# arkworks-rs/algebra

Hardware: AMD Instinct MI355X
Metric: G1 scalar-muls/sec (MSM, 2^24) (higher is better)
Workload: dtype u32

## Files before the change

algebra_amd/_lib.py:

```python
import ctypes as C
import os

_HERE = os.path.dirname(os.path.abspath(__file__))
LIB_PATH = os.environ.get("ARK_HIP_LIB") or os.path.join(_HERE, "libark_hip.so")

u64p = C.POINTER(C.c_uint64)


class ArkHipError(RuntimeError):
    def __init__(self, code, what):
        super().__init__("%s failed with code %d" % (what, code))
        self.code = code


class Radix2DomainStruct(C.Structure):
    _fields_ = [
        ("size", C.c_uint64),
        ("log_size_of_group", C.c_uint32),
        ("_pad", C.c_uint32),
        ("size_as_field_element", C.c_uint64 * 4),
        ("size_inv", C.c_uint64 * 4),
        ("group_gen", C.c_uint64 * 4),
        ("group_gen_inv", C.c_uint64 * 4),
        ("offset", C.c_uint64 * 4),
# ... 131 lines not shown
    "ark_hip_test_host_sw_check": (C.c_int, [C.c_int, C.c_void_p, C.c_size_t, C.c_int, C.c_int, C.c_void_p]),
    "ark_hip_test_host_sw_decompress": (C.c_int, [C.c_int, C.c_void_p, C.c_size_t, C.c_int, C.c_int, C.c_void_p, C.c_void_p]),
    "ark_hip_test_host_sw_compress": (C.c_int, [C.c_int, C.c_void_p, C.c_size_t, C.c_void_p]),
    "ark_hip_test_host_sw_mul": (C.c_int, [C.c_int, C.c_void_p, C.c_int, C.c_void_p, C.c_size_t, C.c_int, C.c_int, C.c_size_t, C.c_void_p]),
    "ark_hip_test_host_sw_add": (C.c_int, [C.c_int, C.c_void_p, C.c_void_p, C.c_int, C.c_size_t, C.c_void_p]),
    "ark_hip_test_host_sw_fold": (C.c_int, [C.c_int, C.c_void_p, C.c_void_p, C.c_int, C.c_void_p, C.c_void_p, C.c_int, C.c_int, C.c_size_t,
                                            C.c_void_p]),
    "ark_hip_test_coord_sqrt": (C.c_int, [C.c_int, C.c_void_p, C.c_void_p, C.c_void_p, C.c_size_t]),
    "ark_hip_test_host_coord_sqrt": (C.c_int, [C.c_int, C.c_void_p, C.c_void_p, C.c_void_p, C.c_size_t]),
    "ark_hip_test_point_op": (C.c_int, [C.c_int, C.c_int, C.c_void_p, C.c_void_p, C.c_void_p, C.c_size_t]),
    "ark_hip_test_msm_sharded_emulated": (C.c_int, [C.c_int, C.c_int, C.POINTER(C.c_void_p), C.POINTER(C.c_void_p),
                                                    C.POINTER(C.c_size_t), C.c_int, C.c_void_p, C.POINTER(C.c_int)]),
    "ark_hip_test_base_hash": (C.c_int, [C.c_void_p, C.c_size_t, C.POINTER(C.c_uint64)]),
    "ark_hip_test_lazy_raw_op": (C.c_int, [C.c_int, C.c_int, C.c_int, C.c_int, C.c_void_p, C.c_void_p, C.c_size_t]),
    "ark_hip_test_lazy_acc_op": (C.c_int, [C.c_int, C.c_int, C.c_void_p, C.c_void_p, C.c_void_p, C.c_size_t]),
    "ark_hip_test_relaxed_raw_op": (C.c_int, [C.c_int, C.c_int, C.c_void_p, C.c_void_p, C.c_size_t]),
    "ark_hip_test_relaxed_acc_op": (C.c_int, [C.c_int, C.c_int, C.c_void_p, C.c_void_p, C.c_void_p, C.c_size_t]),
    "ark_hip_test_msm_host_fold": (C.c_int, [C.c_int, C.c_void_p, C.c_int, C.c_int, C.c_int, C.c_void_p, C.c_void_p]),
    "ark_hip_test_msm_reduce_geometry": (C.c_int, [C.c_int, C.c_int, C.c_int, C.c_int, C.c_int, C.c_size_t, C.POINTER(C.c_uint32)]),
    "ark_hip_test_msm_sort_geometry": (C.c_int, [C.c_int, C.c_size_t, C.c_int, C.c_int, C.c_int, C.c_int, C.POINTER(C.c_int32),
                                                 C.POINTER(C.c_uint64)]),
    "ark_hip_test_msm_sort_stages": (C.c_int, [C.c_int, C.c_void_p, C.c_int, C.c_size_t, C.c_int, C.c_int, C.c_int,
                                               C.POINTER(C.c_int32), C.POINTER(C.c_uint64), C.POINTER(C.c_void_p),
                                               C.POINTER(C.c_size_t)]),
    "ark_hip_test_msm_pieces": (C.c_int, [C.c_int, C.c_void_p, C.c_void_p, C.c_int, C.c_size_t, C.c_int, C.POINTER(C.c_size_t), C.c_int,
                                          C.POINTER(C.c_int32), C.POINTER(C.c_uint64), C.c_void_p, C.c_size_t, C.c_void_p, C.c_size_t,
                                          C.c_void_p]),
    "ark_hip_test_msm_host_fold_l0": (C.c_int, [C.c_int, C.c_void_p, C.c_int, C.c_int, C.c_int, C.c_void_p, C.c_void_p]),
}

# ... 66 lines not shown
```

algebra_amd/csrc/curve_consts.hpp:

```cpp
#pragma once
#include <stdint.h>
namespace arkhip {
static const uint64_t GEN_BN254_G1[8] = {0xd35d438dc58f0d9dULL, 0x0a78eb28f5c70b3dULL, 0x666ea36f7879462cULL, 0x0e0a77c19a07df2fULL, 0xa6ba871b8b1e1b3aULL, 0x14f1d651eb8e167bULL, 0xccdd46def0f28c58ULL, 0x1c14ef83340fbe5eULL};
static const uint64_t GEN_BLS12_381_G1[12] = {0x5cb38790fd530c16ULL, 0x7817fc679976fff5ULL, 0x154f95c7143ba1c1ULL, 0xf0ae6acdf3d0e747ULL, 0xedce6ecc21dbf440ULL, 0x120177419e0bfb75ULL, 0xbaac93d50ce72271ULL, 0x8c22631a7918fd8eULL, 0xdd595f13570725ceULL, 0x51ac582950405194ULL, 0x0e1c8c3fad0059c0ULL, 0x0bbc3efc5008a26aULL};
static const uint64_t GEN_BLS12_377_G1[12] = {0x260f33b9772451f4ULL, 0xc54dd773169d5658ULL, 0x5c1551c469a510ddULL, 0x761662e4425e1698ULL, 0xc97d78cc6f065272ULL, 0x00a41206b361fd4dULL, 0x8193961fb8cb81f3ULL, 0x00638d4c5f44adb8ULL, 0xfafaf3dad4daf54aULL, 0xc27849e2d655cd18ULL, 0x2ec3ddb401d52814ULL, 0x007da93326303c71ULL};
static const uint64_t GEN_BLS12_377_G2[24] = {0x68904082f268725bULL, 0x668f2ea74f45328bULL, 0xebca7a65802be84fULL, 0x1e1850f4c1ada3e6ULL, 0x830dc22d588ef1e9ULL, 0x01862a81767c0982ULL, 0x5f02a915c91c7f39ULL, 0xf8c553ba388da2a7ULL, 0xd51a416dbd198850ULL, 0xe943c6f38ae3073aULL, 0xffe24aa8259a4981ULL, 0x011853391e73dfddULL, 0xd5b19b897881430fULL, 0x05be9118a5b371edULL, 0x6063f91f86c131eeULL, 0x3244a61be8f4ec19ULL, 0xa02e425b9f9a3a12ULL, 0x018af8c04f3360d2ULL, 0x57601ac71a5b96f5ULL, 0xe99acc1714f2440eULL, 0x2339612f10118ea9ULL, 0x8321e68a3b1cd722ULL, 0x2b543b050cc74917ULL, 0x00590182b396c112ULL};
static const uint64_t GEN_BLS12_381_G2[24] = {0xf5f28fa202940a10ULL, 0xb3f5fb2687b4961aULL, 0xa1a893b53e2ae580ULL, 0x9894999d1a3caee9ULL, 0x6f67b7631863366bULL, 0x058191924350bcd7ULL, 0xa5a9c0759e23f606ULL, 0xaaa0c59dbccd60c3ULL, 0x3bb17e18e2867806ULL, 0x1b1ab6cc8541b367ULL, 0xc2b6ed0ef2158547ULL, 0x11922a097360edf3ULL, 0x4c730af860494c4aULL, 0x597cfa1f5e369c5aULL, 0xe7e6856caa0a635aULL, 0xbbefb5e96e0d495fULL, 0x07d3a975f0ef25a2ULL, 0x0083fd8e7e80dae5ULL, 0xadc0fc92df64b05dULL, 0x18aa270a2b1461dcULL, 0x86adac6a3be4eba0ULL, 0x79495c4ec93da33aULL, 0xe7175850a43ccaedULL, 0x0b2bc2a163de1bf2ULL};
}
```

algebra_amd/csrc/lazyk.cuh:

```cuda
#pragma once
#include "curves.cuh"
#include "ec28.cuh"
#include "ec28x2.cuh"

namespace arkhip {

template <class C, int LANES_ = C::FA::LANES>
struct LazyK;

template <class C>
struct LazyK<C, 1> {
  typedef typename C::F FM;
  typedef typename FM::P P;
  typedef FpL<P> FL;
  typedef XYZZL<P> Acc;
  static constexpr u32 LANES = 1;
  static constexpr int WORDS = 4 * FL::L + 1;
  ARK_HD static Acc inf() {
    Acc a;
    a.inf = true;
    a.x = a.y = a.zz = a.zzz = FL::zero();
    return a;
  }
  ARK_HD static Acc from_bucket(const XYZZ<FM>& b) { return lazy_from_bucket<P>(b); }
// ... 24 lines not shown
    const u32* w = (const u32*)slot;
    Acc a;
#pragma unroll
    for (int i = 0; i < FL::L; i++) {
      a.x.l[i] = w[i];
      a.y.l[i] = w[FL::L + i];
      a.zz.l[i] = w[2 * FL::L + i];
      a.zzz.l[i] = w[3 * FL::L + i];
    }
    a.inf = w[4 * FL::L] != 0u;
    return a;
  }
};

template <class C>
struct LazyK<C, 2> {
  typedef typename C::FA FM;
  typedef typename FM::P P;
  typedef Fp2L<P, FM::NEG_BETA_> FL;
  typedef XYZZL2<FL> Acc;
  static constexpr u32 LANES = 2;
  static constexpr int L = FL::L;
  static constexpr int WORDS = 8 * L + 1;
  ARK_DEV static Acc inf() { return lazy2_inf<FL>(); }
  ARK_DEV static Acc from_bucket(const XYZZ<FM>& b) { return lazy2_from_bucket<FL>(b); }
  ARK_DEV static XYZZ<FM> to_bucket(const Acc& a) { return lazy2_to_bucket<FL>(a); }
  ARK_DEV static bool madd(Acc& acc, const Affine<FM>& p, bool neg) {
    return xyzz_madd_lazy2<FL>(acc, FL::from_canonical(p.x), FL::from_canonical(FM::cond_neg(p.y, neg)));
  }
  ARK_DEV static void mdbl(Acc& out, const char* src, bool neg) { lazy2_mdbl<FL>(out, src, neg); }
// ... 33 lines not shown
```

algebra_amd/csrc/msm.cuh:

```cuda
#pragma once
#include <hip/hip_runtime.h>
#include <stdio.h>
#include <stdlib.h>
#include <vector>
#include <mutex>
#include <atomic>
#include "hostpool.hpp"
#include <math.h>
#include "curves.cuh"
#include "ec28.cuh"
#include "lazyk.cuh"
#include "msm_sort.cuh"
#include "msm_plan.hpp"

namespace arkhip {

#define ARK_HIP_TRY(expr)                                                                          \
  do {                                                                                             \
    hipError_t _e = (expr);                                                                        \
    if (_e != hipSuccess) {                                                                        \
      fprintf(stderr, "ark_hip: %s failed: %s (%s:%d)\n", #expr, hipGetErrorString(_e), __FILE__, __LINE__); \
      return -(int)_e - 1000;                                                                      \
    }                                                                                              \
  } while (0)
// ... 441 lines not shown
  }
  if constexpr (C::RELAXED_A) acc = xyzz_canonical<F>(acc);
  acc.store(cell);
}

#ifndef ARK_LAZY_MIN_WAVES
#define ARK_LAZY_MIN_WAVES 2
#endif
template <class C>
__global__ void __launch_bounds__(256, ARK_LAZY_MIN_WAVES) msm_accumulate_lazy_kernel(const char* __restrict__ bases,
                                                                  const u32* __restrict__ sorted,
                                                                  const u32* __restrict__ offsets,
                                                                  const u32* __restrict__ order, u32 nbuckets,
                                                                  const u32* __restrict__ d_thresh, int HB, int LB,
                                                                  int accum, char* __restrict__ buckets) {
  typedef LazyK<C> K;
  typedef typename K::FM F;
  u32 t = (blockIdx.x * blockDim.x + threadIdx.x) / K::LANES;
  if (t >= nbuckets) return;
  u32 g = order ? order[t] : t;
  u32 j = offsets[g], end = offsets[g + 1];
  if (end - j > *d_thresh) return;
  if (accum && j == end) return;
  char* cell = buckets + (size_t)msm_slot_to_bucket(g, HB, LB) * XYZZ<F>::BYTES;
  typename K::Acc acc = K::inf();
  if (accum) acc = K::from_bucket(XYZZ<F>::load(cell));
  if (j < end) {
    u32 e = sorted[j];
    u32 e1 = j + 1 < end ? sorted[j + 1] : 0;
    Affine<F> p = Affine<F>::load(bases + (size_t)(e & 0x7fffffffu) * Affine<F>::BYTES);
    for (;;) {
// ... 1494 lines not shown
```

algebra_amd/csrc/testops_curve.hip:

```cpp
#include "devops.cuh"
#include "testops.cuh"
#include "lazytest.cuh"
#include "relaxtest.cuh"
#include "pointcodec.cuh"
#include "internal.hpp"
#ifndef ARK_TEST_CURVE
#error "compile with -DARK_TEST_CURVE=BLS12_381_G1 (or another curve of curves.cuh)"
#endif
#define ARK_CAT2(a, b) a##b
#define ARK_CAT(a, b) ARK_CAT2(a, b)
namespace arkhip {
int ARK_CAT(test_basefield_op_, ARK_TEST_CURVE)(int op, const void* a, const void* b, void* r, size_t n, hipStream_t s) {
  return field_op_launch<ARK_TEST_CURVE::F, false>(op, a, b, r, n, s);
}
int ARK_CAT(test_point_op_, ARK_TEST_CURVE)(int kind, const void* acc, const void* other, void* out, size_t n, hipStream_t s) {
  return test_point_op_launch<ARK_TEST_CURVE>(kind, acc, other, out, n, s);
}
int ARK_CAT(test_coord_sqrt_, ARK_TEST_CURVE)(const void* in, void* out, void* ok, size_t n, hipStream_t s) {
  return coord_sqrt_launch<ARK_TEST_CURVE>(in, out, ok, n, s);
}
int ARK_CAT(test_lazy_raw_op_, ARK_TEST_CURVE)(int op, int k, int h, const void* in, void* out, size_t n, hipStream_t s) {
  typedef LazyK<ARK_TEST_CURVE> K;
  if constexpr (K::LANES == 1) return lazytest::lazy_raw_op_launch<typename K::P, false, void>(op, k, h, in, out, n, s);
  else return lazytest::lazy_raw_op_launch<typename K::P, false, typename K::FL>(op, k, h, in, out, n, s);
}
int ARK_CAT(test_lazy_acc_op_, ARK_TEST_CURVE)(int kind, const void* acc, const void* other, void* out, size_t n, hipStream_t s) {
  return lazytest::lazy_acc_op_launch<ARK_TEST_CURVE>(kind, acc, other, out, n, s);
}
int ARK_CAT(test_relaxed_raw_op_, ARK_TEST_CURVE)(int op, const void* in, void* out, size_t n, hipStream_t s) {
  typedef ARK_TEST_CURVE::FA FA;
  return relaxtest::relaxed_raw_op_launch<FA::P, relaxtest::NegBetaOf<FA>::v>(op, in, out, n, s);
}
int ARK_CAT(test_relaxed_acc_op_, ARK_TEST_CURVE)(int kind, const void* acc, const void* other, void* out, size_t n, hipStream_t s) {
  return relaxtest::relaxed_acc_op_launch<ARK_TEST_CURVE>(kind, acc, other, out, n, s);
}
}
```

algebra_amd/csrc/ubench/issuebench.hip:

```cpp
#include <hip/hip_runtime.h>
#include <stdint.h>
#include <stdio.h>
typedef uint32_t u32;
typedef uint64_t u64;

#define R8(X) X X X X X X X X
#define KERNEL32(NAME, I0, I1, I2, I3)                                                                        \
  __global__ void __launch_bounds__(256) NAME(u64* out, int iters) {                                         \
    u32 tid = blockIdx.x * blockDim.x + threadIdx.x;                                                          \
    u32 a0 = tid, a1 = tid + 1, a2 = tid + 2, a3 = tid + 3;                                                   \
    const u32 x = tid * 2654435761u | 0x80000001u, y = (tid * 40503u + 7u) | 0x80000000u;                     \
    for (int k = 0; k < iters; k++)                                                                           \
      asm volatile(R8(I0 "\n\t" I1 "\n\t" I2 "\n\t" I3 "\n\t") : "+v"(a0), "+v"(a1), "+v"(a2), "+v"(a3) : "v"(x), "v"(y) : "vcc"); \
    out[tid] = a0 ^ a1 ^ a2 ^ a3;                                                                             \
  }
#define KERNEL64(NAME, T, TX, I0, I1, I2, I3)                                                                     \
  __global__ void __launch_bounds__(256) NAME(u64* out, int iters) {                                         \
    u32 tid = blockIdx.x * blockDim.x + threadIdx.x;                                                          \
    T a0 = (T)tid, a1 = (T)(tid + 1), a2 = (T)(tid + 2), a3 = (T)(tid + 3);                                   \
    const TX x = (TX)(tid | 1u), y = (TX)((tid * 40503u + 7u) | 0x80000000u);                                    \
    for (int k = 0; k < iters; k++)                                                                           \
      asm volatile(R8(I0 "\n\t" I1 "\n\t" I2 "\n\t" I3 "\n\t") : "+v"(a0), "+v"(a1), "+v"(a2), "+v"(a3) : "v"(x), "v"(y) : "vcc"); \
    T s = a0 + a1 + a2 + a3;                                                                                  \
    out[tid] = *(u64*)&s;                                                                                     \
  }
KERNEL32(k_add32, "v_add_u32 %0, %4, %0", "v_add_u32 %1, %4, %1", "v_add_u32 %2, %4, %2", "v_add_u32 %3, %4, %3")
KERNEL32(k_mad24, "v_mad_u32_u24 %0, %4, %5, %0", "v_mad_u32_u24 %1, %4, %5, %1", "v_mad_u32_u24 %2, %4, %5, %2", "v_mad_u32_u24 %3, %4, %5, %3")
KERNEL32(k_mulhi24, "v_mul_hi_u32_u24 %0, %4, %0", "v_mul_hi_u32_u24 %1, %4, %1", "v_mul_hi_u32_u24 %2, %4, %2", "v_mul_hi_u32_u24 %3, %4, %3")
KERNEL32(k_mullo32, "v_mul_lo_u32 %0, %4, %0", "v_mul_lo_u32 %1, %4, %1", "v_mul_lo_u32 %2, %4, %2", "v_mul_lo_u32 %3, %4, %3")
KERNEL32(k_mulhi32, "v_mul_hi_u32 %0, %4, %0", "v_mul_hi_u32 %1, %4, %1", "v_mul_hi_u32 %2, %4, %2", "v_mul_hi_u32 %3, %4, %3")
KERNEL32(k_addc, "v_add_co_u32 %0, vcc, %4, %0", "v_addc_co_u32 %1, vcc, %5, %1, vcc", "v_add_co_u32 %2, vcc, %4, %2", "v_addc_co_u32 %3, vcc, %5, %3, vcc")
KERNEL64(k_mad64, u64, u32, "v_mad_u64_u32 %0, vcc, %4, %5, %0", "v_mad_u64_u32 %1, vcc, %4, %5, %1", "v_mad_u64_u32 %2, vcc, %4, %5, %2", "v_mad_u64_u32 %3, vcc, %4, %5, %3")
KERNEL64(k_add64, u64, u64, "v_lshl_add_u64 %0, %4, 0, %0", "v_lshl_add_u64 %1, %4, 0, %1", "v_lshl_add_u64 %2, %4, 0, %2", "v_lshl_add_u64 %3, %4, 0, %3")
KERNEL64(k_fma64, double, double, "v_fma_f64 %0, %4, %5, %0", "v_fma_f64 %1, %4, %5, %1", "v_fma_f64 %2, %4, %5, %2", "v_fma_f64 %3, %4, %5, %3")
KERNEL64(k_mul64f, double, double, "v_mul_f64 %0, %4, %0", "v_mul_f64 %1, %4, %1", "v_mul_f64 %2, %4, %2", "v_mul_f64 %3, %4, %3")

typedef void (*kern_t)(u64*, int);
int main() {
  u64* out;
  if (hipMalloc(&out, 256 * 8 * 256 * 8) != hipSuccess) return 1;
  hipEvent_t e0, e1;
  hipEventCreate(&e0);
  hipEventCreate(&e1);
  struct { const char* name; kern_t k; } ks[] = {
      {"v_add_u32            ", k_add32},  {"v_mad_u32_u24        ", k_mad24},   {"v_mul_hi_u32_u24     ", k_mulhi24},
      {"v_mul_lo_u32         ", k_mullo32}, {"v_mul_hi_u32         ", k_mulhi32}, {"v_add_co + v_addc_co ", k_addc},
      {"v_mad_u64_u32        ", k_mad64},  {"v_lshl_add_u64       ", k_add64},   {"v_fma_f64            ", k_fma64},
      {"v_mul_f64            ", k_mul64f}};
  for (auto& e : ks) {
    for (int w : {2, 8}) {
      const int b = 256 * w, it = 4000;
      hipLaunchKernelGGL(e.k, dim3(b), dim3(256), 0, 0, out, 10);
      hipDeviceSynchronize();
      hipEventRecord(e0);
      hipLaunchKernelGGL(e.k, dim3(b), dim3(256), 0, 0, out, it);
      hipEventRecord(e1);
      hipEventSynchronize(e1);
      float ms;
      hipEventElapsedTime(&ms, e0, e1);
      const double rate = (double)b * 256 * it * 32 / (ms * 1e-3);
      printf("%s waves/SIMD=%d  %8.3f ms  %7.2f T lane-ops/s  = %5.2f cycles per wave instruction at 2.4 GHz\n", e.name, w, ms,
             rate * 1e-12, 256.0 * 4 * 64 * 2.4e9 / rate);
// ... 5 lines not shown
```

algebra_amd/csrc/ubench/mulbench.hip:

```cpp
#include "../fp28.cuh"
#include <stdio.h>
using namespace arkhip;
#ifndef MULBENCH_FIELD
#define MULBENCH_FIELD BLS12_381_FQ
#endif
typedef MULBENCH_FIELD P;
template <int V> __global__ void __launch_bounds__(256) k_lazy(u32* out, int iters) {
  typedef FpL<P> L;
  L a, b;
  u32 tid = blockIdx.x * blockDim.x + threadIdx.x;
  for (int i = 0; i < L::L; i++) { a.l[i] = (tid * 2654435761u * (i + 1)) & L::MASK; b.l[i] = ((tid ^ 77) * 40503u * (i + 3)) & L::MASK; }
  a.l[L::L - 1] &= 0xfff; b.l[L::L - 1] &= 0xfff;
  for (int k = 0; k < iters; k++) {
    if constexpr (V == 0) a = L::mul_c(a, b);
    else if constexpr (V == 1) a = L::mul(a, b);
    else if constexpr (V == 2) a = L::sqr(a);
    else if constexpr (V == 3) a = L::sop2(a, b, b, a);
    else a = L::sqr_c(a);
  }
  u32 r = 0;
  for (int i = 0; i < L::L; i++) r ^= a.l[i];
  out[tid] = r;
}
__global__ void __launch_bounds__(256) k_sat(u32* out, int iters) {
  typedef Fp<P> F;
  F a, b;
  u32 tid = blockIdx.x * blockDim.x + threadIdx.x;
  for (int i = 0; i < F::N; i++) { a.l[i] = (tid * 2654435761u * (i + 1)); b.l[i] = ((tid ^ 77) * 40503u * (i + 3)); }
  a.l[F::N - 1] &= 0x7ffffff; b.l[F::N - 1] &= 0x7ffffff;
  for (int k = 0; k < iters; k++) a = F::mul(a, b);
  u32 r = 0;
  for (int i = 0; i < F::N; i++) r ^= a.l[i];
  out[tid] = r;
}
__global__ void __launch_bounds__(256) k_mad_peak(u64* out, int iters, u32 mask) {
  u32 tid = blockIdx.x * blockDim.x + threadIdx.x;
  u64 a0 = tid, a1 = tid + 1, a2 = tid + 2, a3 = tid + 3;
  const u32 x = (tid * 2654435761u | 0x80000001u) & mask, y = ((tid * 40503u + 7u) | 0x80000000u) & mask;
// ... 38 lines not shown
          case 4: hipLaunchKernelGGL((k_lazy<4>), dim3(b), dim3(256), 0, 0, out, it); break;
          default: hipLaunchKernelGGL(k_sat, dim3(b), dim3(256), 0, 0, out, it);
        }
      };
      launch(10);
      hipDeviceSynchronize();
      hipEventRecord(e0);
      launch(iters);
      hipEventRecord(e1);
      hipEventSynchronize(e1);
      float ms;
      hipEventElapsedTime(&ms, e0, e1);
      printf("%s waves/SIMD=%d  %8.3f ms  %8.2f G/s\n", names[v], w, ms, (double)b * 256 * iters / (ms * 1e-3) * 1e-9);
    }
  }
  return 0;
}
```

include/ark_hip.h:

```cpp
#ifndef ARK_HIP_H
#define ARK_HIP_H
#include <stddef.h>
#include <stdint.h>
#ifdef __cplusplus
extern "C" {
#endif
#if defined(__GNUC__) || defined(__clang__)
#pragma GCC visibility push(default)
#endif

enum { ARK_HIP_BN254_FQ = 0, ARK_HIP_BN254_FR = 1, ARK_HIP_BLS12_381_FQ = 2, ARK_HIP_BLS12_381_FR = 3,
       ARK_HIP_BLS12_377_FQ = 4, ARK_HIP_BLS12_377_FR = 5 };
enum { ARK_HIP_BN254_G1 = 0, ARK_HIP_BLS12_381_G1 = 1, ARK_HIP_BLS12_377_G1 = 2, ARK_HIP_BLS12_377_G2 = 3,
       ARK_HIP_BLS12_381_G2 = 4 };
enum { ARK_HIP_OK = 0, ARK_HIP_ERR_ARG = -1, ARK_HIP_ERR_SIZE = -2, ARK_HIP_ERR_NOMEM = -3,
       ARK_HIP_ERR_SCALAR_RANGE = -4, ARK_HIP_ERR_NO_DEVICE = -5, ARK_HIP_ERR_BUSY = -6,
       ARK_HIP_ERR_COMM = -7   };

int ark_hip_device_count(void);
int ark_hip_init(int device);
int ark_hip_set_device(int device);
int ark_hip_get_device(void);
void ark_hip_shutdown(void);
int ark_hip_synchronize(void);
// ... 188 lines not shown
                                      const size_t* n_local, int scalars_are_montgomery, uint64_t* out_xyz, int* path);
int ark_hip_test_base_hash(const uint64_t* p, size_t words, uint64_t out[2]);
int ark_hip_test_msm_host_fold(int curve, const uint64_t* parts, int windows, int nbits, int log2_l0, const int* widths,
                               uint64_t* out_xyz);
int ark_hip_test_msm_host_fold_l0(int curve, const uint64_t* parts, int windows, int nbits, int l0, const int* widths,
                                  uint64_t* out_xyz);
int ark_hip_test_msm_reduce_geometry(int curve, int c, int W, int narrow, int shared, size_t resident_lanes, uint32_t out[12]);
int ark_hip_test_msm_sort_geometry(int curve, size_t n, int c, int W, int narrow, int shared, const int32_t knobs[8], uint64_t out[32]);
int ark_hip_test_msm_sort_stages(int curve, const void* scalars, int on_device, size_t n, int mont, int sbytes, int sbits,
                                 const int32_t knobs[8], uint64_t header[32], void* const* out, const size_t* cap_words);
int ark_hip_test_msm_pieces(int curve, const void* bases, const void* scalars, int on_device, size_t n, int mont, const size_t* sizes,
                            int npieces, const int32_t knobs[12], uint64_t header[80], uint32_t* hctr_out, size_t hctr_cap_words,
                            void* buckets_out, size_t buckets_cap_bytes, uint64_t* out_xyz);
int ark_hip_test_lazy_raw_op(int field, int op, int k, int h, const uint32_t* in, uint32_t* out, size_t n);
int ark_hip_test_lazy_acc_op(int curve, int kind, const void* acc, const void* other, void* out, size_t n);
int ark_hip_test_relaxed_raw_op(int field, int op, const uint32_t* in, uint32_t* out, size_t n);
int ark_hip_test_relaxed_acc_op(int curve, int kind, const void* acc, const void* other, void* out, size_t n);
typedef struct ark_hip_scratch_row {
  char name[40];
  uint64_t cap, asked, regrown, dirty_beyond, first_dirty_offset;
} ark_hip_scratch_row;
int ark_hip_test_scratch_poison(uint32_t word);
int ark_hip_test_scratch_report(uint32_t word, ark_hip_scratch_row* rows, size_t cap_rows, size_t* n_rows);
int ark_hip_test_scratch_selfcheck(void);

#endif

#if defined(__GNUC__) || defined(__clang__)
#pragma GCC visibility pop
#endif
// ... 5 lines not shown
```

Measured before the change: 476.3 million.

## Add signed 13x30-bit digit Montgomery arithmetic for BLS12-381 bucket accumulation

Adds a field representation for BLS12-381 Fq that uses 13 signed 30-bit digits, multiplied with v_mad_i64_i32 inline asm, in place of 14 unsigned 28-bit limbs. It also adds an XYZZ mixed-add built on it and a LazySK accumulator enabled by default through ARK_LAZY_S30. The aim is fewer limb products per Montgomery multiply in the MSM bucket-accumulation inner loop. The cost is extra conversions to and from the canonical form and more involved signed carry handling with tight bounds. Test entry points and microbenchmarks are added as well.

```diff
diff --git a/algebra_amd/_lib.py b/algebra_amd/_lib.py
--- a/algebra_amd/_lib.py
+++ b/algebra_amd/_lib.py
@@ -169,6 +169,7 @@
     "ark_hip_test_base_hash": (C.c_int, [C.c_void_p, C.c_size_t, C.POINTER(C.c_uint64)]),
     "ark_hip_test_lazy_raw_op": (C.c_int, [C.c_int, C.c_int, C.c_int, C.c_int, C.c_void_p, C.c_void_p, C.c_size_t]),
     "ark_hip_test_lazy_acc_op": (C.c_int, [C.c_int, C.c_int, C.c_void_p, C.c_void_p, C.c_void_p, C.c_size_t]),
+    "ark_hip_test_s30_op": (C.c_int, [C.c_int, C.c_void_p, C.c_void_p, C.c_size_t]),
     "ark_hip_test_relaxed_raw_op": (C.c_int, [C.c_int, C.c_int, C.c_void_p, C.c_void_p, C.c_size_t]),
     "ark_hip_test_relaxed_acc_op": (C.c_int, [C.c_int, C.c_int, C.c_void_p, C.c_void_p, C.c_void_p, C.c_size_t]),
     "ark_hip_test_msm_host_fold": (C.c_int, [C.c_int, C.c_void_p, C.c_int, C.c_int, C.c_int, C.c_void_p, C.c_void_p]),
diff --git a/algebra_amd/csrc/curve_consts.hpp b/algebra_amd/csrc/curve_consts.hpp
--- a/algebra_amd/csrc/curve_consts.hpp
+++ b/algebra_amd/csrc/curve_consts.hpp
@@ -6,4 +6,12 @@
 static const uint64_t GEN_BLS12_377_G1[12] = {0x260f33b9772451f4ULL, 0xc54dd773169d5658ULL, 0x5c1551c469a510ddULL, 0x761662e4425e1698ULL, 0xc97d78cc6f065272ULL, 0x00a41206b361fd4dULL, 0x8193961fb8cb81f3ULL, 0x00638d4c5f44adb8ULL, 0xfafaf3dad4daf54aULL, 0xc27849e2d655cd18ULL, 0x2ec3ddb401d52814ULL, 0x007da93326303c71ULL};
 static const uint64_t GEN_BLS12_377_G2[24] = {0x68904082f268725bULL, 0x668f2ea74f45328bULL, 0xebca7a65802be84fULL, 0x1e1850f4c1ada3e6ULL, 0x830dc22d588ef1e9ULL, 0x01862a81767c0982ULL, 0x5f02a915c91c7f39ULL, 0xf8c553ba388da2a7ULL, 0xd51a416dbd198850ULL, 0xe943c6f38ae3073aULL, 0xffe24aa8259a4981ULL, 0x011853391e73dfddULL, 0xd5b19b897881430fULL, 0x05be9118a5b371edULL, 0x6063f91f86c131eeULL, 0x3244a61be8f4ec19ULL, 0xa02e425b9f9a3a12ULL, 0x018af8c04f3360d2ULL, 0x57601ac71a5b96f5ULL, 0xe99acc1714f2440eULL, 0x2339612f10118ea9ULL, 0x8321e68a3b1cd722ULL, 0x2b543b050cc74917ULL, 0x00590182b396c112ULL};
 static const uint64_t GEN_BLS12_381_G2[24] = {0xf5f28fa202940a10ULL, 0xb3f5fb2687b4961aULL, 0xa1a893b53e2ae580ULL, 0x9894999d1a3caee9ULL, 0x6f67b7631863366bULL, 0x058191924350bcd7ULL, 0xa5a9c0759e23f606ULL, 0xaaa0c59dbccd60c3ULL, 0x3bb17e18e2867806ULL, 0x1b1ab6cc8541b367ULL, 0xc2b6ed0ef2158547ULL, 0x11922a097360edf3ULL, 0x4c730af860494c4aULL, 0x597cfa1f5e369c5aULL, 0xe7e6856caa0a635aULL, 0xbbefb5e96e0d495fULL, 0x07d3a975f0ef25a2ULL, 0x0083fd8e7e80dae5ULL, 0xadc0fc92df64b05dULL, 0x18aa270a2b1461dcULL, 0x86adac6a3be4eba0ULL, 0x79495c4ec93da33aULL, 0xe7175850a43ccaedULL, 0x0b2bc2a163de1bf2ULL};
+struct S30_BLS12_381_FQ {
+  static constexpr int W = 30, L = 13;
+  static constexpr int32_t P[13] = {-21845, -402915328, 356515836, -352321620, -252304353, 55215067, 288093811, 316751073, -321428361, 517541167, -375082566, -91332614, 1704210};
+  static constexpr uint32_t INV = 0x3ffcfffdu;
+  static constexpr int32_t ONE[13] = {13762350, 433586176, -192935228, -301937177, 37952645, -425753694, -36732706, 162803105, -437337492, 366579475, 78814996, -442511456, 89578};
+  static constexpr int OUT_K = 4;
+  static constexpr int32_t OUT_KP[13] = {-87380, 535822336, 352321518, -335544655, 64524411, 220860267, 78633420, 193262469, -211971619, -77318981, -426588438, -365330457, 6816840};
+};
 }
diff --git a/algebra_amd/csrc/ec30s.cuh b/algebra_amd/csrc/ec30s.cuh
--- /dev/null
+++ b/algebra_amd/csrc/ec30s.cuh
@@ -0,0 +1,81 @@
+#pragma once
+#include "ec28.cuh"
+#include "fp30s.cuh"
+
+namespace arkhip {
+
+template <class P>
+struct XYZZS {
+  FpS<P> x, y, zz, zzz;
+  bool inf;
+};
+
+template <class P>
+ARK_HD void s30_from_affine(const Fp<P>& x, const Fp<P>& y, FpS<P>& xs, FpS<P>& ys) {
+  xs = FpS<P>::from_canonical_shl(x.l);
+  ys = FpS<P>::from_canonical_shl(y.l);
+}
+template <class P>
+ARK_HD XYZZS<P> s30_from_bucket(const XYZZ<Fp<P>>& b) {
+  typedef FpS<P> F;
+  XYZZS<P> r;
+  r.inf = b.is_zero();
+  const F one = F::one();
+  r.x = F::mul(F::from_canonical_shl(b.x.l), one);
+  r.y = F::mul(F::from_canonical_shl(b.y.l), one);
+  r.zz = F::mul(F::from_canonical_shl(b.zz.l), one);
+  r.zzz = F::mul(F::from_canonical_shl(b.zzz.l), one);
+  return r;
+}
+template <class P>
+ARK_HD XYZZ<Fp<P>> s30_to_bucket(const XYZZS<P>& a) {
+  if (a.inf) return XYZZ<Fp<P>>::zero();
+  XYZZ<Fp<P>> r;
+  r.x = a.x.to_canonical();
+  r.y = a.y.to_canonical();
+  r.zz = a.zz.to_canonical();
+  r.zzz = a.zzz.to_canonical();
+  return r;
+}
+template <class P>
+ARK_COLD_HD void xyzz_mdbl_s(XYZZS<P>& acc, const char* src, bool neg) {
+  XYZZL<P> d;
+  xyzz_mdbl_lazy<P>(d, src, neg);
+  acc = s30_from_bucket<P>(lazy_to_bucket<P>(d));
+}
+
+template <class P>
+ARK_HD bool xyzz_madd_s(XYZZS<P>& acc, const FpS<P>& x2, const FpS<P>& y2) {
+  typedef FpS<P> F;
+  if (acc.inf) {
+    const F one = F::one();
+    acc.x = F::mul(x2, one);
+    acc.y = F::mul(y2, one);
+    acc.zz = one;
+    acc.zzz = one;
+    acc.inf = false;
+    return false;
+  }
+  const F u2 = F::mul(x2, acc.zz);
+  const F s2 = F::mul(y2, acc.zzz);
+  const F pd = F::sub(u2, acc.x);
+  const F rd = F::sub(s2, acc.y);
+  const F pp = F::sqr(pd);
+  if (pp.is_zero_digits()) {
+    if (F::sqr(rd).is_zero_digits()) return true;
+    acc.inf = true;
+    return false;
+  }
+  const F ppp = F::mul(pd, pp);
+  const F q = F::mul(acc.x, pp);
+  const F e = F::add_2b(ppp, q);
+  const F x3 = F::sub(F::sqr(rd), e);
+  const F t = F::sub(q, x3);
+  acc.y = F::sop2(rd, t, F::neg(acc.y), ppp);
+  acc.zz = F::mul(acc.zz, pp);
+  acc.zzz = F::mul(acc.zzz, ppp);
+  acc.x = x3;
+  return false;
+}
+
+}
diff --git a/algebra_amd/csrc/fp30s.cuh b/algebra_amd/csrc/fp30s.cuh
--- /dev/null
+++ b/algebra_amd/csrc/fp30s.cuh
@@ -0,0 +1,311 @@
+#pragma once
+#include "curve_consts.hpp"
+#include "fp.cuh"
+
+namespace arkhip {
+
+typedef int32_t i32;
+typedef int64_t i64;
+
+template <class P> struct S30Of;
+template <> struct S30Of<BLS12_381_FQ> { typedef S30_BLS12_381_FQ T; };
+
+#define ARK_SMA(A, B) "v_mad_i64_i32 %0, vcc, %" #A ", %" #B ", %0\n\t"
+#define ARK_ST1 ARK_SMA(1, 2)
+#define ARK_ST2 ARK_ST1 ARK_SMA(3, 4)
+#define ARK_ST3 ARK_ST2 ARK_SMA(5, 6)
+#define ARK_ST4 ARK_ST3 ARK_SMA(7, 8)
+#define ARK_ST5 ARK_ST4 ARK_SMA(9, 10)
+#define ARK_ST6 ARK_ST5 ARK_SMA(11, 12)
+#define ARK_ST7 ARK_ST6 ARK_SMA(13, 14)
+#define ARK_ST8 ARK_ST7 ARK_SMA(15, 16)
+#define ARK_ST9 ARK_ST8 ARK_SMA(17, 18)
+#define ARK_ST10 ARK_ST9 ARK_SMA(19, 20)
+#define ARK_ST11 ARK_ST10 ARK_SMA(21, 22)
+#define ARK_ST12 ARK_ST11 ARK_SMA(23, 24)
+#define ARK_ST13 ARK_ST12 ARK_SMA(25, 26)
+#define ARK_SOP(i) "v"(x[LO + i]), "s"(PSD<S, K - LO - i>::v)
+#define ARK_SOP1 ARK_SOP(0)
+#define ARK_SOP2 ARK_SOP1, ARK_SOP(1)
+#define ARK_SOP3 ARK_SOP2, ARK_SOP(2)
+#define ARK_SOP4 ARK_SOP3, ARK_SOP(3)
+#define ARK_SOP5 ARK_SOP4, ARK_SOP(4)
+#define ARK_SOP6 ARK_SOP5, ARK_SOP(5)
+#define ARK_SOP7 ARK_SOP6, ARK_SOP(6)
+#define ARK_SOP8 ARK_SOP7, ARK_SOP(7)
+#define ARK_SOP9 ARK_SOP8, ARK_SOP(8)
+#define ARK_SOP10 ARK_SOP9, ARK_SOP(9)
+#define ARK_SOP11 ARK_SOP10, ARK_SOP(10)
+#define ARK_SOP12 ARK_SOP11, ARK_SOP(11)
+#define ARK_SOP13 ARK_SOP12, ARK_SOP(12)
+#define ARK_SSTMT(n, OPS) \
+  if constexpr (HIX - LO + 1 == n) asm(ARK_ST##n : "+v"(c) : OPS##n : "vcc")
+#define ARK_SALL(OPS)                                                                                       \
+  ARK_SSTMT(1, OPS); ARK_SSTMT(2, OPS); ARK_SSTMT(3, OPS); ARK_SSTMT(4, OPS); ARK_SSTMT(5, OPS); ARK_SSTMT(6, OPS); \
+  ARK_SSTMT(7, OPS); ARK_SSTMT(8, OPS); ARK_SSTMT(9, OPS); ARK_SSTMT(10, OPS); ARK_SSTMT(11, OPS); ARK_SSTMT(12, OPS); \
+  ARK_SSTMT(13, OPS)
+template <class S, int I> struct PSD { static constexpr i32 v = S::P[I]; };
+template <int LO, int HIX, int K>
+ARK_DEV void scol_vv(i64& c, const i32* x, const i32* y) {
+  if constexpr (HIX >= LO) { ARK_SALL(ARK_OV); }
+}
+template <class S, int LO, int HIX, int K>
+ARK_DEV void scol_vp(i64& c, const i32* x) {
+  if constexpr (HIX >= LO) { ARK_SALL(ARK_SOP); }
+}
+
+template <class P_>
+struct FpS {
+  typedef P_ P;
+  typedef typename S30Of<P>::T S;
+  static constexpr int L = S::L;
+  static constexpr int W = S::W;
+  static constexpr int N = P::N;
+  static constexpr int SH = W * L - 32 * N;
+  static constexpr i32 HALF = 1 << (W - 1);
+  static_assert(W == 30 && L == 13 && SH > 0 && SH < 8, "bounds in this file are written for 13 x 30 bits");
+  i32 l[L];
+
+  ARK_HD static i32 digit(u32 v) { return (i32)(v << (32 - W)) >> (32 - W); }
+  ARK_HD static u64 prod(i32 a, i32 b) { return (u64)((i64)a * (i64)b); }
+
+  ARK_HD static FpS zero() {
+    FpS r;
+#pragma unroll
+    for (int i = 0; i < L; i++) r.l[i] = 0;
+    return r;
+  }
+  ARK_HD static FpS one() {
+    FpS r;
+#pragma unroll
+    for (int i = 0; i < L; i++) r.l[i] = S::ONE[i];
+    return r;
+  }
+
+  template <int NP>
+  ARK_HD static FpS mont_c(const i32* a, const i32* b, const i32* x, const i32* y) {
+    i32 m[L];
+    FpS r;
+    u64 t = 0;
+#pragma unroll
+    for (int k = 0; k < 2 * L - 1; k++) {
+      const int lo = k < L ? 0 : k - L + 1, hi = k < L ? k : L - 1;
+#pragma unroll
+      for (int i = lo; i <= hi; i++) {
+        t += prod(a[i], b[k - i]);
+        if constexpr (NP == 2) t += prod(x[i], y[k - i]);
+      }
+#pragma unroll
+      for (int i = lo; i <= (k < L ? k - 1 : L - 1); i++) t += prod(m[i], S::P[k - i]);
+      if (k < L) {
+        m[k] = digit((u32)t * S::INV);
+        t += prod(m[k], S::P[0]);
+      } else {
+        r.l[k - L] = digit((u32)t);
+        t += (u64)HALF;
+      }
+      t = (u64)((i64)t >> W);
+    }
+    r.l[L - 1] = (i32)(u32)t;
+    return r;
+  }
+  ARK_HD static FpS mul_c(const FpS& a, const FpS& b) { return mont_c<1>(a.l, b.l, nullptr, nullptr); }
+  ARK_HD static FpS sop2_c(const FpS& a, const FpS& b, const FpS& x, const FpS& y) { return mont_c<2>(a.l, b.l, x.l, y.l); }
+  ARK_HD static FpS sqr_c(const FpS& a) {
+    i32 m[L], d[L];
+    FpS r;
+#pragma unroll
+    for (int i = 0; i < L; i++) d[i] = (i32)((u32)a.l[i] << 1);
+    u64 t = 0;
+#pragma unroll
+    for (int k = 0; k < 2 * L - 1; k++) {
+      const int lo = k < L ? 0 : k - L + 1;
+#pragma unroll
+      for (int i = lo; 2 * i < k; i++) t += prod(a.l[i], d[k - i]);
+      if (k % 2 == 0) t += prod(a.l[k / 2], a.l[k / 2]);
+#pragma unroll
+      for (int i = lo; i <= (k < L ? k - 1 : L - 1); i++) t += prod(m[i], S::P[k - i]);
+      if (k < L) {
+        m[k] = digit((u32)t * S::INV);
+        t += prod(m[k], S::P[0]);
+      } else {
+        r.l[k - L] = digit((u32)t);
+        t += (u64)HALF;
+      }
+      t = (u64)((i64)t >> W);
+    }
+    r.l[L - 1] = (i32)(u32)t;
+    return r;
+  }
+
+#if defined(__HIP_DEVICE_COMPILE__)
+  template <int K, int NP>
+  ARK_DEV static void s_cols_lo(i64& c, const i32* a, const i32* b, const i32* x, const i32* y, i32* m) {
+    scol_vv<0, K, K>(c, a, b);
+    if constexpr (NP >= 2) scol_vv<0, K, K>(c, x, y);
+    scol_vp<S, 0, K - 1, K>(c, m);
+    m[K] = digit((u32)c * S::INV);
+    scol_vp<S, K, K, K>(c, m);
+    c >>= W;
+    if constexpr (K + 1 < L) s_cols_lo<K + 1, NP>(c, a, b, x, y, m);
+  }
+  template <int K, int NP>
+  ARK_DEV static void s_cols_hi(i64& c, const i32* a, const i32* b, const i32* x, const i32* y, const i32* m, i32* r) {
+    scol_vv<K - L + 1, L - 1, K>(c, a, b);
+    if constexpr (NP >= 2) scol_vv<K - L + 1, L - 1, K>(c, x, y);
+    scol_vp<S, K - L + 1, L - 1, K>(c, m);
+    r[K - L] = digit((u32)c);
+    c = (c + HALF) >> W;
+    if constexpr (K + 1 < 2 * L - 1) s_cols_hi<K + 1, NP>(c, a, b, x, y, m, r);
+  }
+  template <int K>
+  ARK_DEV static void s_sq_lo(i64& c, const i32* a, const i32* d, i32* m) {
+    if constexpr (K >= 1) scol_vv<0, (K - 1) / 2, K>(c, a, d);
+    if constexpr (K % 2 == 0) scol_vv<K / 2, K / 2, K>(c, a, a);
+    scol_vp<S, 0, K - 1, K>(c, m);
+    m[K] = digit((u32)c * S::INV);
+    scol_vp<S, K, K, K>(c, m);
+    c >>= W;
+    if constexpr (K + 1 < L) s_sq_lo<K + 1>(c, a, d, m);
+  }
+  template <int K>
+  ARK_DEV static void s_sq_hi(i64& c, const i32* a, const i32* d, const i32* m, i32* r) {
+    scol_vv<K - L + 1, (K - 1) / 2, K>(c, a, d);
+    if constexpr (K % 2 == 0) scol_vv<K / 2, K / 2, K>(c, a, a);
+    scol_vp<S, K - L + 1, L - 1, K>(c, m);
+    r[K - L] = digit((u32)c);
+    c = (c + HALF) >> W;
+    if constexpr (K + 1 < 2 * L - 1) s_sq_hi<K + 1>(c, a, d, m, r);
+  }
+  ARK_DEV static FpS mul(const FpS& a, const FpS& b) {
+    i32 m[L];
+    FpS r;
+    i64 c = 0;
+    s_cols_lo<0, 1>(c, a.l, b.l, nullptr, nullptr, m);
+    s_cols_hi<L, 1>(c, a.l, b.l, nullptr, nullptr, m, r.l);
+    r.l[L - 1] = (i32)c;
+    return r;
+  }
+  ARK_DEV static FpS sop2(const FpS& a, const FpS& b, const FpS& x, const FpS& y) {
+    i32 m[L];
+    FpS r;
+    i64 c = 0;
+    s_cols_lo<0, 2>(c, a.l, b.l, x.l, y.l, m);
+    s_cols_hi<L, 2>(c, a.l, b.l, x.l, y.l, m, r.l);
+    r.l[L - 1] = (i32)c;
+    return r;
+  }
+  ARK_DEV static FpS sqr(const FpS& a) {
+    i32 m[L], d[L];
+    FpS r;
+#pragma unroll
+    for (int i = 0; i < L; i++) d[i] = (i32)((u32)a.l[i] << 1);
+    i64 c = 0;
+    s_sq_lo<0>(c, a.l, d, m);
+    s_sq_hi<L>(c, a.l, d, m, r.l);
+    r.l[L - 1] = (i32)c;
+    return r;
+  }
+#else
+  static FpS mul(const FpS& a, const FpS& b) { return mul_c(a, b); }
+  static FpS sqr(const FpS& a) { return sqr_c(a); }
+  static FpS sop2(const FpS& a, const FpS& b, const FpS& x, const FpS& y) { return sop2_c(a, b, x, y); }
+#endif
+
+  template <bool WIDE = false>
+  ARK_HD static FpS sweep(const i32* d) {
+    FpS r;
+    i32 carry = 0;
+#pragma unroll
+    for (int i = 0; i < L - 1; i++) {
+      const i32 v = d[i] + carry;
+      r.l[i] = digit((u32)v);
+      if constexpr (WIDE) carry = ((v >> 1) + (HALF >> 1)) >> (W - 1);
+      else carry = (v + HALF) >> W;
+    }
+    r.l[L - 1] = d[L - 1] + carry;
+    return r;
+  }
+  ARK_HD static FpS sub(const FpS& a, const FpS& b) {
+    i32 d[L];
+#pragma unroll
+    for (int i = 0; i < L; i++) d[i] = a.l[i] - b.l[i];
+    return sweep(d);
+  }
+  ARK_HD static FpS add_2b(const FpS& a, const FpS& b) {
+    i32 d[L];
+#pragma unroll
+    for (int i = 0; i < L; i++) d[i] = a.l[i] + 2 * b.l[i];
+    return sweep<true>(d);
+  }
+  ARK_HD static FpS add(const FpS& a, const FpS& b) {
+    i32 d[L];
+#pragma unroll
+    for (int i = 0; i < L; i++) d[i] = a.l[i] + b.l[i];
+    return sweep(d);
+  }
+  ARK_HD static FpS neg(const FpS& a) {
+    FpS r;
+#pragma unroll
+    for (int i = 0; i < L; i++) r.l[i] = -a.l[i];
+    return r;
+  }
+  ARK_HD bool is_zero_digits() const {
+    u32 o = 0;
+#pragma unroll
+    for (int i = 0; i < L; i++) o |= (u32)l[i];
+    return o == 0u;
+  }
+
+  ARK_HD static FpS from_canonical_shl(const u32* in) {
+    FpS r;
+    u32 carry = 0;
+#pragma unroll
+    for (int i = 0; i < L; i++) {
+      const int bit = W * i - SH;
+      u32 u;
+      if (bit < 0) {
+        u = (in[0] << SH) & ((1u << W) - 1u);
+      } else {
+        const int j = bit / 32, sh = bit % 32;
+        u64 v = 0;
+        if (j < N) v = (u64)in[j] >> sh;
+        if (j + 1 < N) v |= (u64)in[j + 1] << (32 - sh);
+        u = (u32)v & ((1u << W) - 1u);
+      }
+      u += carry;
+      if (i < L - 1) {
+        r.l[i] = digit(u);
+        carry = (u + (u32)HALF) >> W;
+      } else {
+        r.l[i] = (i32)u;
+      }
+    }
+    return r;
+  }
+  ARK_HD Fp<P> to_canonical() const {
+    const u32 w0 = (u32)l[0] + (u32)S::OUT_KP[0];
+    const u32 m = (w0 * S::INV) & ((1u << SH) - 1u);
+    u32 t[L];
+    i64 acc = 0;
+#pragma unroll
+    for (int i = 0; i < L; i++) {
+      acc += (i64)l[i] + (i64)S::OUT_KP[i] + (i64)m * (i64)S::P[i];
+      t[i] = (u32)acc & ((1u << W) - 1u);
+      acc >>= W;
+    }
+    u32 out[N];
+#pragma unroll
+    for (int j = 0; j < N; j++) {
+      const int bit = 32 * j + SH;
+      const int i = bit / W, sh = bit % W;
+      u64 v = (u64)t[i] >> sh;
+      if (i + 1 < L) v |= (u64)t[i + 1] << (W - sh);
+      if (i + 2 < L) v |= (u64)t[i + 2] << (2 * W - sh);
+      out[j] = (u32)v;
+    }
+    return Fp<P>::reduce_once(out);
+  }
+};
+
+}
diff --git a/algebra_amd/csrc/lazyk.cuh b/algebra_amd/csrc/lazyk.cuh
--- a/algebra_amd/csrc/lazyk.cuh
+++ b/algebra_amd/csrc/lazyk.cuh
@@ -2,6 +2,12 @@
 #include "curves.cuh"
 #include "ec28.cuh"
 #include "ec28x2.cuh"
+#include "ec30s.cuh"
+#include <type_traits>
+
+#ifndef ARK_LAZY_S30
+#define ARK_LAZY_S30 1
+#endif
 
 namespace arkhip {
 
@@ -62,6 +68,60 @@
 };
 
 template <class C>
+struct LazySK {
+  typedef typename C::F FM;
+  typedef typename FM::P P;
+  typedef FpS<P> FL;
+  typedef XYZZS<P> Acc;
+  static constexpr u32 LANES = 1;
+  static constexpr int WORDS = 4 * FL::L + 1;
+  ARK_HD static Acc inf() {
+    Acc a;
+    a.inf = true;
+    a.x = a.y = a.zz = a.zzz = FL::zero();
+    return a;
+  }
+  ARK_HD static Acc from_bucket(const XYZZ<FM>& b) { return s30_from_bucket<P>(b); }
+  ARK_HD static XYZZ<FM> to_bucket(const Acc& a) { return s30_to_bucket<P>(a); }
+  ARK_HD static bool madd(Acc& acc, const Affine<FM>& p, bool neg) {
+    FL sx, sy;
+    s30_from_affine<P>(p.x, FM::cond_neg(p.y, neg), sx, sy);
+    return xyzz_madd_s<P>(acc, sx, sy);
+  }
+  ARK_HD static void mdbl(Acc& out, const char* src, bool neg) { xyzz_mdbl_s<P>(out, src, neg); }
+  ARK_HD static void park(const Acc& a, i32* w) {
+#pragma unroll
+    for (int i = 0; i < FL::L; i++) {
+      w[i] = a.x.l[i];
+      w[FL::L + i] = a.y.l[i];
+      w[2 * FL::L + i] = a.zz.l[i];
+      w[3 * FL::L + i] = a.zzz.l[i];
+    }
+    w[4 * FL::L] = a.inf ? 1 : 0;
+  }
+  ARK_HD static Acc unpark(const i32* w) {
+    Acc a;
+#pragma unroll
+    for (int i = 0; i < FL::L; i++) {
+      a.x.l[i] = w[i];
+      a.y.l[i] = w[FL::L + i];
+      a.zz.l[i] = w[2 * FL::L + i];
+      a.zzz.l[i] = w[3 * FL::L + i];
+    }
+    a.inf = w[4 * FL::L] != 0;
+    return a;
+  }
+};
+template <class P, class = void> struct HasS30 : std::false_type {};
+template <class P> struct HasS30<P, std::void_t<typename S30Of<P>::T>> : std::true_type {};
+template <class C, int LANES_ = C::FA::LANES, class = void>
+struct AccumK { typedef LazyK<C> T; };
+#if ARK_LAZY_S30
+template <class C>
+struct AccumK<C, 1, std::enable_if_t<HasS30<typename C::F::P>::value>> { typedef LazySK<C> T; };
+#endif
+
+template <class C>
 struct LazyK<C, 2> {
   typedef typename C::FA FM;
   typedef typename FM::P P;
diff --git a/algebra_amd/csrc/msm.cuh b/algebra_amd/csrc/msm.cuh
--- a/algebra_amd/csrc/msm.cuh
+++ b/algebra_amd/csrc/msm.cuh
@@ -479,7 +479,7 @@
                                                                   const u32* __restrict__ order, u32 nbuckets,
                                                                   const u32* __restrict__ d_thresh, int HB, int LB,
                                                                   int accum, char* __restrict__ buckets) {
-  typedef LazyK<C> K;
+  typedef typename AccumK<C>::T K;
   typedef typename K::FM F;
   u32 t = (blockIdx.x * blockDim.x + threadIdx.x) / K::LANES;
   if (t >= nbuckets) return;
diff --git a/algebra_amd/csrc/s30test.cuh b/algebra_amd/csrc/s30test.cuh
--- /dev/null
+++ b/algebra_amd/csrc/s30test.cuh
@@ -0,0 +1,79 @@
+#pragma once
+#include "curves.cuh"
+#include "lazyk.cuh"
+#include "s30test_api.hpp"
+
+namespace arkhip {
+namespace s30test {
+
+template <class C>
+ARK_HD void s30_raw_apply(int op, const i32* in, i32* out) {
+  typedef LazySK<C> K;
+  typedef typename K::FL F;
+  typedef typename K::FM FM;
+  static_assert(F::L == SLOT, "slot = 13 digits");
+  auto ld = [&](int j) {
+    F x;
+#pragma unroll
+    for (int i = 0; i < SLOT; i++) x.l[i] = in[j * SLOT + i];
+    return x;
+  };
+  auto canon = [&](int at) {
+    FM x;
+#pragma unroll
+    for (int i = 0; i < FM::N; i++) x.l[i] = (u32)in[at + i];
+    return x;
+  };
+  F r = F::zero();
+  switch (op) {
+    case MUL: r = F::mul(ld(0), ld(1)); break;
+    case SQR: r = F::sqr(ld(0)); break;
+    case SOP2: r = F::sop2(ld(0), ld(1), ld(2), ld(3)); break;
+    case SUB: r = F::sub(ld(0), ld(1)); break;
+    case ADD_2B: r = F::add_2b(ld(0), ld(1)); break;
+    case FROM_CANONICAL_SHL: r = F::from_canonical_shl(canon(0).l); break;
+    case TO_CANONICAL: {
+      const FM c = ld(0).to_canonical();
+#pragma unroll
+      for (int i = 0; i < FM::N; i++) r.l[i] = (i32)c.l[i];
+      break;
+    }
+    case MADD: {
+      typename K::Acc acc = K::unpark(in);
+      F x2, y2;
+      s30_from_affine<typename K::P>(canon(4 * SLOT + 1), canon(5 * SLOT + 1), x2, y2);
+      const bool eq = xyzz_madd_s<typename K::P>(acc, x2, y2);
+      K::park(acc, out);
+      out[4 * SLOT + 1] = eq ? 1 : 0;
+      return;
+    }
+    default: break;
+  }
+#pragma unroll
+  for (int i = 0; i < SLOT; i++) out[i] = r.l[i];
+}
+
+template <class C, int LN = C::FA::LANES> struct Served : std::false_type {};
+template <class C> struct Served<C, 1> : HasS30<typename C::F::P> {};
+
+#if defined(__HIPCC__)
+template <class C>
+__global__ void __launch_bounds__(128) s30_raw_op_kernel(int op, const i32* __restrict__ in, i32* __restrict__ out, size_t n) {
+  const size_t t = (size_t)blockIdx.x * blockDim.x + threadIdx.x;
+  if (t >= n) return;
+  s30_raw_apply<C>(op, in + t * (size_t)in_words(op), out + t * (size_t)out_words(op));
+}
+template <class C>
+int s30_raw_op_launch(int op, const void* in, void* out, size_t n, hipStream_t s) {
+  if constexpr (Served<C>::value) {
+    if (op < 0 || op >= OPS) return -1;
+    hipLaunchKernelGGL((s30_raw_op_kernel<C>), dim3((unsigned)((n + 127) / 128)), dim3(128), 0, s, op, (const i32*)in, (i32*)out, n);
+    return hipGetLastError() == hipSuccess ? 0 : -1000;
+  } else {
+    return -1;
+  }
+}
+#endif
+
+}
+}
diff --git a/algebra_amd/csrc/s30test_api.hpp b/algebra_amd/csrc/s30test_api.hpp
--- /dev/null
+++ b/algebra_amd/csrc/s30test_api.hpp
@@ -0,0 +1,26 @@
+#pragma once
+#include <stddef.h>
+#include <stdint.h>
+
+namespace arkhip {
+namespace s30test {
+
+enum Op : int {
+  MUL = 0,
+  SQR = 1,
+  SOP2 = 2,
+  SUB = 3,
+  ADD_2B = 4,
+  FROM_CANONICAL_SHL = 5,
+  TO_CANONICAL = 6,
+  MADD = 7,
+  OPS = 8
+};
+constexpr int SLOT = 13;
+constexpr int in_words(int op) {
+  return op == MADD ? 4 * SLOT + 1 + 2 * SLOT : SLOT * (op == MUL || op == SUB || op == ADD_2B ? 2 : (op == SOP2 ? 4 : 1));
+}
+constexpr int out_words(int op) { return op == MADD ? 4 * SLOT + 2 : SLOT; }
+
+}
+}
diff --git a/algebra_amd/csrc/testops_curve.hip b/algebra_amd/csrc/testops_curve.hip
--- a/algebra_amd/csrc/testops_curve.hip
+++ b/algebra_amd/csrc/testops_curve.hip
@@ -2,6 +2,7 @@
 #include "testops.cuh"
 #include "lazytest.cuh"
 #include "relaxtest.cuh"
+#include "s30test.cuh"
 #include "pointcodec.cuh"
 #include "internal.hpp"
 #ifndef ARK_TEST_CURVE
@@ -27,6 +28,9 @@
 int ARK_CAT(test_lazy_acc_op_, ARK_TEST_CURVE)(int kind, const void* acc, const void* other, void* out, size_t n, hipStream_t s) {
   return lazytest::lazy_acc_op_launch<ARK_TEST_CURVE>(kind, acc, other, out, n, s);
 }
+int ARK_CAT(test_s30_raw_op_, ARK_TEST_CURVE)(int op, const void* in, void* out, size_t n, hipStream_t s) {
+  return s30test::s30_raw_op_launch<ARK_TEST_CURVE>(op, in, out, n, s);
+}
 int ARK_CAT(test_relaxed_raw_op_, ARK_TEST_CURVE)(int op, const void* in, void* out, size_t n, hipStream_t s) {
   typedef ARK_TEST_CURVE::FA FA;
   return relaxtest::relaxed_raw_op_launch<FA::P, relaxtest::NegBetaOf<FA>::v>(op, in, out, n, s);
diff --git a/algebra_amd/csrc/ubench/issuebench.hip b/algebra_amd/csrc/ubench/issuebench.hip
--- a/algebra_amd/csrc/ubench/issuebench.hip
+++ b/algebra_amd/csrc/ubench/issuebench.hip
@@ -31,6 +31,7 @@
 KERNEL32(k_mulhi32, "v_mul_hi_u32 %0, %4, %0", "v_mul_hi_u32 %1, %4, %1", "v_mul_hi_u32 %2, %4, %2", "v_mul_hi_u32 %3, %4, %3")
 KERNEL32(k_addc, "v_add_co_u32 %0, vcc, %4, %0", "v_addc_co_u32 %1, vcc, %5, %1, vcc", "v_add_co_u32 %2, vcc, %4, %2", "v_addc_co_u32 %3, vcc, %5, %3, vcc")
 KERNEL64(k_mad64, u64, u32, "v_mad_u64_u32 %0, vcc, %4, %5, %0", "v_mad_u64_u32 %1, vcc, %4, %5, %1", "v_mad_u64_u32 %2, vcc, %4, %5, %2", "v_mad_u64_u32 %3, vcc, %4, %5, %3")
+KERNEL64(k_madi64, int64_t, int32_t, "v_mad_i64_i32 %0, vcc, %4, %5, %0", "v_mad_i64_i32 %1, vcc, %4, %5, %1", "v_mad_i64_i32 %2, vcc, %4, %5, %2", "v_mad_i64_i32 %3, vcc, %4, %5, %3")
 KERNEL64(k_add64, u64, u64, "v_lshl_add_u64 %0, %4, 0, %0", "v_lshl_add_u64 %1, %4, 0, %1", "v_lshl_add_u64 %2, %4, 0, %2", "v_lshl_add_u64 %3, %4, 0, %3")
 KERNEL64(k_fma64, double, double, "v_fma_f64 %0, %4, %5, %0", "v_fma_f64 %1, %4, %5, %1", "v_fma_f64 %2, %4, %5, %2", "v_fma_f64 %3, %4, %5, %3")
 KERNEL64(k_mul64f, double, double, "v_mul_f64 %0, %4, %0", "v_mul_f64 %1, %4, %1", "v_mul_f64 %2, %4, %2", "v_mul_f64 %3, %4, %3")
@@ -45,7 +46,7 @@
   struct { const char* name; kern_t k; } ks[] = {
       {"v_add_u32            ", k_add32},  {"v_mad_u32_u24        ", k_mad24},   {"v_mul_hi_u32_u24     ", k_mulhi24},
       {"v_mul_lo_u32         ", k_mullo32}, {"v_mul_hi_u32         ", k_mulhi32}, {"v_add_co + v_addc_co ", k_addc},
-      {"v_mad_u64_u32        ", k_mad64},  {"v_lshl_add_u64       ", k_add64},   {"v_fma_f64            ", k_fma64},
+      {"v_mad_u64_u32        ", k_mad64},  {"v_mad_i64_i32        ", k_madi64}, {"v_lshl_add_u64       ", k_add64},   {"v_fma_f64            ", k_fma64},
       {"v_mul_f64            ", k_mul64f}};
   for (auto& e : ks) {
     for (int w : {2, 8}) {
diff --git a/algebra_amd/csrc/ubench/mulbench.hip b/algebra_amd/csrc/ubench/mulbench.hip
--- a/algebra_amd/csrc/ubench/mulbench.hip
+++ b/algebra_amd/csrc/ubench/mulbench.hip
@@ -3,6 +3,11 @@
 using namespace arkhip;
 #ifndef MULBENCH_FIELD
 #define MULBENCH_FIELD BLS12_381_FQ
+#define MULBENCH_S30 1
+#include "../fp30s.cuh"
+#endif
+#ifndef MULBENCH_REPEATS
+#define MULBENCH_REPEATS 7
 #endif
 typedef MULBENCH_FIELD P;
 template <int V> __global__ void __launch_bounds__(256) k_lazy(u32* out, int iters) {
@@ -22,6 +27,25 @@
   for (int i = 0; i < L::L; i++) r ^= a.l[i];
   out[tid] = r;
 }
+#ifdef MULBENCH_S30
+template <int V> __global__ void __launch_bounds__(256) k_s30(u32* out, int iters) {
+  typedef FpS<P> S;
+  S a, b;
+  u32 tid = blockIdx.x * blockDim.x + threadIdx.x;
+  for (int i = 0; i < S::L; i++) { a.l[i] = S::digit(tid * 2654435761u * (i + 1)); b.l[i] = S::digit((tid ^ 77) * 40503u * (i + 3)); }
+  a.l[S::L - 1] >>= 9; b.l[S::L - 1] >>= 9;
+  for (int k = 0; k < iters; k++) {
+    if constexpr (V == 0) a = S::mul_c(a, b);
+    else if constexpr (V == 1) a = S::mul(a, b);
+    else if constexpr (V == 2) a = S::sqr(a);
+    else if constexpr (V == 3) a = S::sop2(a, b, b, a);
+    else a = S::sub(S::mul(a, b), S::mul(b, a));
+  }
+  u32 r = 0;
+  for (int i = 0; i < S::L; i++) r ^= (u32)a.l[i];
+  out[tid] = r;
+}
+#endif
 __global__ void __launch_bounds__(256) k_sat(u32* out, int iters) {
   typedef Fp<P> F;
   F a, b;
@@ -90,5 +114,44 @@
       printf("%s waves/SIMD=%d  %8.3f ms  %8.2f G/s\n", names[v], w, ms, (double)b * 256 * iters / (ms * 1e-3) * 1e-9);
     }
   }
+#ifdef MULBENCH_S30
+  printf("13 x 30-bit signed digits (v_mad_i64_i32) against 14 x 28-bit limbs (v_mad_u64_u32), waves/SIMD=2, %d alternated repeats\n", MULBENCH_REPEATS);
+  const char* gn[8] = {"lazy28 mul ", "signed30 mul ", "lazy28 sqr ", "signed30 sqr ", "lazy28 sop2", "signed30 sop2", "signed30 mul, portable", "signed30 two mul + sub"};
+  double lo[8], hi[8], sum[8];
+  for (int v = 0; v < 8; v++) { lo[v] = 1e30; hi[v] = 0; sum[v] = 0; }
+  for (int rep = 0; rep < MULBENCH_REPEATS; rep++) {
+    for (int v = 0; v < 8; v++) {
+      const int b = 256 * 2;
+      auto launch = [&](int it) {
+        switch (v) {
+          case 0: hipLaunchKernelGGL((k_lazy<1>), dim3(b), dim3(256), 0, 0, out, it); break;
+          case 1: hipLaunchKernelGGL((k_s30<1>), dim3(b), dim3(256), 0, 0, out, it); break;
+          case 2: hipLaunchKernelGGL((k_lazy<2>), dim3(b), dim3(256), 0, 0, out, it); break;
+          case 3: hipLaunchKernelGGL((k_s30<2>), dim3(b), dim3(256), 0, 0, out, it); break;
+          case 4: hipLaunchKernelGGL((k_lazy<3>), dim3(b), dim3(256), 0, 0, out, it); break;
+          case 5: hipLaunchKernelGGL((k_s30<3>), dim3(b), dim3(256), 0, 0, out, it); break;
+          case 6: hipLaunchKernelGGL((k_s30<0>), dim3(b), dim3(256), 0, 0, out, it); break;
+          default: hipLaunchKernelGGL((k_s30<4>), dim3(b), dim3(256), 0, 0, out, it);
+        }
+      };
+      launch(10);
+      hipDeviceSynchronize();
+      hipEventRecord(e0);
+      launch(iters);
+      hipEventRecord(e1);
+      hipEventSynchronize(e1);
+      float ms;
+      hipEventElapsedTime(&ms, e0, e1);
+      const double g = (double)b * 256 * iters / (ms * 1e-3) * 1e-9;
+      printf("repeat %d  %-24s %8.3f ms  %8.2f G/s\n", rep, gn[v], ms, g);
+      lo[v] = g < lo[v] ? g : lo[v]; hi[v] = g > hi[v] ? g : hi[v]; sum[v] += g;
+    }
+  }
+  for (int v = 0; v < 8; v++)
+    printf("%-24s mean %8.2f G/s  min %8.2f  max %8.2f  spread %5.2f %%\n", gn[v], sum[v] / MULBENCH_REPEATS, lo[v], hi[v],
+           100.0 * (hi[v] - lo[v]) / (sum[v] / MULBENCH_REPEATS));
+  for (int v = 0; v < 6; v += 2)
+    printf("factor %s: signed30 / lazy28 = %.4f (means)\n", gn[v], sum[v + 1] / sum[v]);
+#endif
   return 0;
 }
diff --git a/include/ark_hip.h b/include/ark_hip.h
--- a/include/ark_hip.h
+++ b/include/ark_hip.h
@@ -226,6 +226,7 @@
                             void* buckets_out, size_t buckets_cap_bytes, uint64_t* out_xyz);
 int ark_hip_test_lazy_raw_op(int field, int op, int k, int h, const uint32_t* in, uint32_t* out, size_t n);
 int ark_hip_test_lazy_acc_op(int curve, int kind, const void* acc, const void* other, void* out, size_t n);
+int ark_hip_test_s30_op(int op, const void* in, void* out, size_t n);
 int ark_hip_test_relaxed_raw_op(int field, int op, const uint32_t* in, uint32_t* out, size_t n);
 int ark_hip_test_relaxed_acc_op(int curve, int kind, const void* acc, const void* other, void* out, size_t n);
 typedef struct ark_hip_scratch_row {
```

Result: faster. 482.1 million, median of 6 (+1.2%).
